# 0411tony/Yue

Measured on AMD Instinct MI355X. Metric: BPR triplet-updates/sec at k=128 (S-round semantics, user rows sequential; the reference's exact sequential semantics: secondary.exact), higher is better.
Workload: dtype f32

## Files before the change

yue_amd/csrc/bpr_device.hpp:

```cpp
#pragma once
#include <hip/hip_runtime.h>
#include <stdint.h>

namespace yue {

constexpr int kNllSlots = 1024;
constexpr int kMaxAttempts = 64;

struct TrainArgs {
    float *P, *Q, *dP, *dQ;
    float *stage;
#ifdef YUE_STAMPS
    unsigned long long *stamps;
#endif
    const int32_t *ev_u, *ev_i;
    int32_t *ev_j;
    const int64_t *indptr;
    const int32_t *indices;
    double *nll_slots;
    int64_t m, n;
    int k;
    float ru, ri;
    double lr;
    uint64_t seed;
// ... 76 lines not shown
    const double r8 = r4 * r4;
    const double c0 = __builtin_fma(b1, r4, b0), c1 = __builtin_fma(a6, r4, b2);
    return __builtin_ldexp(__builtin_fma(c1, r8, c0), (int)n);
}
__device__ __forceinline__ double chain_rcp(double d) {
    double y = __builtin_amdgcn_rcp(d);
    double e = __builtin_fma(-d, y, 1.0);
    y = __builtin_fma(e, y, y);
    e = __builtin_fma(-d, y, 1.0);
    y = __builtin_fma(e, y, y);
    e = __builtin_fma(-d, y, 1.0);
    return __builtin_fma(e, y, y);
}

__device__ __forceinline__ double chain_sigmoid(float x) {
    const double xd = (double)x;
    if (__builtin_fabs(xd) <= 700.0) return chain_rcp(1.0 + chain_exp(-xd));
    return 1.0 / (1.0 + exp(-xd));
}
__device__ __forceinline__ float chain_coef_fast(float x, float lr) {
    return lr * __builtin_amdgcn_rcpf(1.0f + __builtin_amdgcn_exp2f(x * 1.44269502162933349609375f));
}

__device__ __forceinline__ float wave_sum_any(float v) {
    v = v + dpp_mov<0xB1>(v);
    v = v + dpp_mov<0x4E>(v);
    v = v + dpp_mov<0x141>(v);
    v = v + dpp_mov<0x140>(v);
    v = v + __builtin_bit_cast(float, __builtin_amdgcn_update_dpp(0, __builtin_bit_cast(int, v), 0x142, 0xA, 0xF, false));
    v = v + __builtin_bit_cast(float, __builtin_amdgcn_update_dpp(0, __builtin_bit_cast(int, v), 0x143, 0xC, 0xF, false));
    return rdlane(v, 63);
}

struct Elem { float p2, qi2, qj2; };
__device__ __forceinline__ Elem bpr_elem(float p, float qi, float qj, float c, float ru, float ri) {
    const float d = qi - qj;
    const float td = c * d;
    const float p1 = p + td;
    const float tq = c * p1;
    const float qi1 = qi + tq;
    const float qj1 = qj - tq;
    const float rp = ru * p1;
    const float ra = ri * qi1;
    const float rb = ri * qj1;
    Elem o;
    o.p2 = p1 - rp;
    o.qi2 = qi1 - ra;
    o.qj2 = qj1 - rb;
    return o;
}

#define YUE_BLOAD(rs, vo, so) __builtin_bit_cast(float, __builtin_amdgcn_raw_buffer_load_b32((rs), (vo), (so), 0))
#define YUE_BSTORE(val, rs, vo, so) __builtin_amdgcn_raw_buffer_store_b32(__builtin_bit_cast(unsigned, (val)), (rs), (vo), (so), 0)
#define YUE_BLOAD_SC1(rs, vo, so) __builtin_bit_cast(float, __builtin_amdgcn_raw_buffer_load_b32((rs), (vo), (so), 16))
#define YUE_BSTORE_SC1(val, rs, vo, so) __builtin_amdgcn_raw_buffer_store_b32(__builtin_bit_cast(unsigned, (val)), (rs), (vo), (so), 16)
#define YUE_BATOMIC(val, rs, vo, so) __builtin_amdgcn_raw_ptr_buffer_atomic_fadd_f32((val), (rs), (vo), (so), 0)
#ifdef YUE_STAMPS
#define YUE_STAMP(ix, waits) do { asm volatile(waits ::: "memory"); if (a.stamps && lane == 0) a.stamps[(size_t)wave * 8 + (ix)] = wall_clock64(); } while (0)
#else
#define YUE_STAMP(ix, waits) do {} while (0)
#endif
constexpr unsigned kOobOffset = 0x80000000u;
constexpr unsigned long long kTouch = 0x100000001ull;
constexpr int kRsrcFlags = 0x00020000;
constexpr unsigned kStageMax = 4;

constexpr int kHeaderSlack = 16;
template <int TPW>
struct __attribute__((aligned(4))) HeaderBlock { int32_t w[TPW]; };

}
```

yue_amd/csrc/bpr_host.hip:

```cpp
#include "host_common.hpp"

#include "train_kernels.hpp"
#include "round_kernels.hpp"

using yue_host::fail;
using yue_host::kr_of;
static_assert(yue::kNllSlots == yue_host::kNllSlotsHost && yue::kHeaderSlack == yue_host::kHeaderSlackHost, "host_common.hpp mirrors these");

namespace {

yue::TrainArgs make_args(yue_ctx *c, double lr, double regU, double regI) {
    yue::TrainArgs a{};
    a.P = c->P.p; a.Q = c->Q.p; a.dP = c->dP.p; a.dQ = c->dQ.p;
    a.stage = c->Q.p ? c->Q.p + (size_t)c->n * c->k : nullptr;
    a.ev_u = c->ev_u.p; a.ev_i = c->ev_i.p; a.ev_j = c->ev_j.p;
    a.indptr = c->indptr.p; a.indices = c->indices.p;
    a.nll_slots = c->scal.p;
    a.m = c->m; a.n = c->n; a.k = c->k;
    a.lr = lr;
    a.ru = (float)(lr * regU);
    a.ri = (float)(lr * regI);
    a.neg_lo = 0; a.neg_range = (int32_t)c->n;
    return a;
}
// ... 110 lines not shown
    if (c->h_bounds != bounds) {
        HIPCHK(hipStreamSynchronize(c->stream));
        c->h_bounds = bounds;
        HIPCHK(hipMemcpyAsync(c->d_bounds.p, c->h_bounds.data(), (size_t)(R + 1) * sizeof(int64_t), hipMemcpyHostToDevice, c->stream));
    }
    HIPCHK(hipMemsetAsync(c->round_rows.p, 0, (size_t)R * sizeof(unsigned long long), c->stream));
    HIPCHK(c->fold.resize((size_t)(E + 4 * R + 8)));
    yue::MetaArgs ma{};
    ma.ev_i = a.ev_i; ma.ev_j = a.ev_j; ma.bounds = c->d_bounds.p; ma.R = R; ma.n = (int32_t)c->n;
    const bool bucketed = meta_bucketed(c);
    if (bucketed) {
        ma.range = 1 << yue::kBucketShift;
        ma.G = (int32_t)((c->n + ma.range - 1) >> yue::kBucketShift);
        HIPCHK(c->bk_touch.resize((size_t)(2 * E + 2))); HIPCHK(c->bk_ptr.resize((size_t)R * (ma.G + 1)));
        yue::BucketArgs ba{};
        ba.ev_i = a.ev_i; ba.ev_j = a.ev_j; ba.bounds = c->d_bounds.p; ba.R = R; ba.G = ma.G;
        ba.bk_touch = c->bk_touch.p; ba.bk_ptr = c->bk_ptr.p; ba.meta_i = c->meta_i.p; ba.meta_j = c->meta_j.p;
        int cus0 = 0;
        HIPCHK(hipDeviceGetAttribute(&cus0, hipDeviceAttributeMultiprocessorCount, c->device));
        hipLaunchKernelGGL(yue::k_round_bucket, dim3((unsigned)std::min<int64_t>(R, 2 * cus0)), dim3(1024), 0, c->stream, ba);
        ma.bk_touch = c->bk_touch.p; ma.bk_ptr = c->bk_ptr.p;
    } else {
        ma.G = (int32_t)((c->n + kMetaRangeMax - 1) / kMetaRangeMax);
        ma.range = (int32_t)((c->n + ma.G - 1) / ma.G);
    }
    ma.chunk = (ma.range + 1023) / 1024; ma.chunk |= 1;
    int64_t widest = 0;
    for (int64_t r = 0; r < R; ++r) widest = std::max(widest, bounds[(size_t)r + 1] - bounds[(size_t)r]);
    const double mean_touches = 2.0 * (double)widest / (double)std::max<int64_t>(1, c->n);
    const uint32_t stage_auto = (uint32_t)std::min<double>((double)yue::kMetaStageMax, std::max<double>((double)yue::kMetaStageDefault,
                                                         std::ceil(mean_touches * (kr_of(c->k) == 1 ? 4.0 : 2.0))));
    ma.stage_max = !c->staged ? 1u : c->opt_round_stage >= 2 ? (uint32_t)c->opt_round_stage : stage_auto;
    c->last_stage_max = (int)ma.stage_max;
    ma.meta_i = c->meta_i.p; ma.meta_j = c->meta_j.p; ma.round_rows = c->round_rows.p; ma.fold = c->fold.p;
    const size_t lds = (size_t)ma.range * sizeof(uint32_t);
    const void *kfn = bucketed ? (const void *)yue::k_round_meta<true> : (const void *)yue::k_round_meta<false>;
    HIPCHK(hipFuncSetAttribute(kfn, hipFuncAttributeMaxDynamicSharedMemorySize, (int)lds));
    int per_cu = 0, cus = 0;
    if (bucketed) { HIPCHK(hipOccupancyMaxActiveBlocksPerMultiprocessor(&per_cu, yue::k_round_meta<true>, 1024, lds)); }
    else { HIPCHK(hipOccupancyMaxActiveBlocksPerMultiprocessor(&per_cu, yue::k_round_meta<false>, 1024, lds)); }
    HIPCHK(hipDeviceGetAttribute(&cus, hipDeviceAttributeMultiprocessorCount, c->device));
    const int64_t grid = std::max<int64_t>(8, std::min<int64_t>((R * ma.G + 7) / 8 * 8, (int64_t)std::max(per_cu, 1) * cus / 8 * 8));
    if (bucketed) hipLaunchKernelGGL(yue::k_round_meta<true>, dim3((unsigned)grid), dim3(1024), lds, c->stream, ma);
    else
        hipLaunchKernelGGL(yue::k_round_meta<false>, dim3((unsigned)grid), dim3(1024), lds, c->stream, ma);
    HIPCHK(hipGetLastError());
    return YUE_OK;
}

void launch_round_fold(yue_ctx *c, const yue::TrainArgs &a, int64_t e0, int64_t e1, int64_t round_index) {
    yue::FoldArgs f{};
    f.fold = c->fold.p + yue::fold_base(e0, round_index); f.round_rows = c->round_rows.p + round_index; f.Q = a.Q; f.dQ = a.dQ; f.stage = a.stage; f.k = c->k; f.capacity = (uint32_t)((e1 - e0) & ~(int64_t)3);
    const dim3 fgrid((unsigned)std::min<int64_t>(c->opt_fold_blocks, std::max<int64_t>(1, (e1 - e0 + 15) / 16))), block(256);
    switch (kr_of(c->k)) {
        case 1: hipLaunchKernelGGL(yue::k_round_fold<1>, fgrid, block, 0, c->stream, f); break;
        case 2: hipLaunchKernelGGL(yue::k_round_fold<2>, fgrid, block, 0, c->stream, f); break;
        default: hipLaunchKernelGGL(yue::k_round_fold<4>, fgrid, block, 0, c->stream, f); break;
    }
}

int launch_round_m(yue_ctx *c, const yue::TrainArgs &a_in, int64_t e0, int64_t e1, int64_t round_index) {
    yue::RoundMArgs ra{};
    ra.e_begin = e0; ra.e_end = e1; ra.staged = c->staged ? 1 : 0;
    const int tpw = tpw_of(c, true);
    const int64_t waves = (e1 - e0 + tpw - 1) / tpw;
    const int64_t blocks = (waves + 3) / 4;
    if (blocks == 0) return YUE_OK;
    const dim3 grid((unsigned)blocks), block(256);
#ifdef YUE_STAMPS
    yue::TrainArgs a = a_in;
    a.stamps = nullptr;
    if (c->update_launches++ == c->stamp_launch) {
        HIPCHK(c->stamps.resize((size_t)waves * 8));
        HIPCHK(hipMemsetAsync(c->stamps.p, 0, (size_t)waves * 64, c->stream));
        a.stamps = c->stamps.p;
        c->stamp_waves = waves;
    }
#else
    const yue::TrainArgs &a = a_in;
#endif
    const uint32_t *mi = c->meta_i.p, *mj = c->meta_j.p;
    if (c->bigq) {
        switch (kr_of(c->k) * 16 + tpw) {
            case 1 * 16 + 8: hipLaunchKernelGGL((yue::k_round_m<1, 8, true>), grid, block, 0, c->stream, a, ra, a.ev_u, a.ev_i, a.ev_j, mi, mj); break;
            case 2 * 16 + 8: hipLaunchKernelGGL((yue::k_round_m<2, 8, true>), grid, block, 0, c->stream, a, ra, a.ev_u, a.ev_i, a.ev_j, mi, mj); break;
// ... 619 lines not shown
```

yue_amd/csrc/core_host.hip:

```cpp
#include "host_common.hpp"

namespace yue_host {
thread_local std::string g_err;
int fail(int code, const std::string &msg) { g_err = msg; return code; }
}
using yue_host::fail;
void yue_comm_release(yue_ctx *c);

extern "C" {

const char *yue_last_error(void) { return yue_host::g_err.c_str(); }
int yue_version(void) { return 1; }

int yue_ctx_create(int device, yue_ctx **out) {
    if (!out) return fail(YUE_ERR_ARG, "yue_ctx_create: out is NULL");
    int ndev = 0;
    HIPCHK(hipGetDeviceCount(&ndev));
    if (ndev <= 0) return fail(YUE_ERR_HIP, "no HIP device visible: libyue_hip needs an MI355X (no CPU fallback exists)");
    if (device < 0 || device >= ndev) return fail(YUE_ERR_ARG, "device ordinal out of range");
    HIPCHK(hipSetDevice(device));
    yue_ctx *c = new yue_ctx();
    c->device = device;
    const auto init = [c]() -> int {
        HIPCHK(hipStreamCreateWithFlags(&c->stream, hipStreamNonBlocking));
// ... 2 lines not shown
        HIPCHK(hipEventCreateWithFlags(&c->ev_comm, hipEventDisableTiming));
        HIPCHK(hipEventCreate(&c->ev_t_rounds));
        HIPCHK(hipEventCreate(&c->ev_t_comm));
        HIPCHK(hipEventCreate(&c->ev_scan0));
        HIPCHK(hipEventCreate(&c->ev_scan1));
        HIPCHK(c->scal.resize(yue_host::kNllSlotsHost + 8));
        return YUE_OK;
    };
    const int rc = init();
    if (rc) { const std::string msg = yue_host::g_err; (void)yue_ctx_destroy(c); yue_host::g_err = msg; return rc; }
    *out = c;
    return YUE_OK;
}

int yue_ctx_destroy(yue_ctx *c) {
    if (!c) return YUE_OK;
    (void)hipSetDevice(c->device);
    if (c->stream) (void)hipStreamSynchronize(c->stream);
    if (c->comm_stream) (void)hipStreamSynchronize(c->comm_stream);
    yue_comm_release(c);
    if (c->comm_stream) (void)hipStreamDestroy(c->comm_stream);
    if (c->ev_rounds) (void)hipEventDestroy(c->ev_rounds);
    if (c->ev_comm) (void)hipEventDestroy(c->ev_comm);
    if (c->ev_t_rounds) (void)hipEventDestroy(c->ev_t_rounds);
    if (c->ev_t_comm) (void)hipEventDestroy(c->ev_t_comm);
    if (c->ev_scan0) (void)hipEventDestroy(c->ev_scan0);
    if (c->ev_chain0) (void)hipEventDestroy(c->ev_chain0);
    if (c->ev_chain1) (void)hipEventDestroy(c->ev_chain1);
    if (c->ev_scan1) (void)hipEventDestroy(c->ev_scan1);
    for (auto &pr : c->ev_pool) { (void)hipEventDestroy(pr.first); (void)hipEventDestroy(pr.second); }
    c->P.release(); c->Q.release(); c->dP.release(); c->dQ.release(); c->margins.release();
    c->cnt0.release(); c->cnt1.release(); c->cntp0.release(); c->cntp1.release();
    c->tab0.release(); c->tab1.release();
    c->meta_i.release(); c->meta_j.release(); c->round_rows.release(); c->d_bounds.release(); c->fold.release(); c->bk_touch.release(); c->bk_ptr.release();
    c->ev_u.release(); c->ev_i.release(); c->ev_j.release(); c->indices.release(); c->indptr.release();
    c->xu.release(); c->xi.release(); c->xj.release(); c->xk.release(); c->x_loss.release(); c->scal.release();
    c->aU_m.release(); c->aU_v.release(); c->aV_m.release(); c->aV_v.release();
    c->s_users.release(); c->s_ids.release(); c->s_mask_idx.release(); c->s_flags.release();
    c->s_mask_ptr.release(); c->s_scores.release(); c->s_row.release(); c->s_norms.release(); c->s_work.release(); c->s_qb.release(); c->s_masks.release(); c->s_few.release(); c->s_few_ids.release(); c->s_few_scores.release();
    c->fP.release(); c->fBi.release(); c->f_coef.release(); c->f_x.release(); c->f_hist.release(); c->f_scores.release();
    c->f_out_sc.release(); c->fQ.release(); c->f_ptr.release(); c->f_items.release(); c->f_negs.release(); c->f_ids.release(); c->f_flags.release();
    c->f_uq_ptr.release(); c->f_neg_ptr.release(); c->f_uq_items.release(); c->f_loc_i.release(); c->f_loc_j.release();
    c->f_wq.release(); c->f_dQ.release(); c->f_wp.release(); c->f_wb.release(); c->f_dP.release(); c->f_dB.release();
    c->ch_key.release(); c->ch_val.release(); c->ch_key2.release(); c->ch_val2.release(); c->ch_seg.release(); c->ch_ord_i.release(); c->ch_ord_j.release();
    c->ch_head.release(); c->ch_incl.release(); c->ch_ord_u.release(); c->ch_rkey.release(); c->ch_rval.release(); c->ch_run_ptr.release(); c->d_ev_ptr.release();
    c->ch_run_u.release(); c->ch_tmp.release(); c->ch_Qv.release(); c->ch_Pv.release(); c->ch_ctl.release(); c->ch_stats.release();
    yue_host::wrmf_release(c);
    yue_host::knn_release(c);
    if (c->stream) (void)hipStreamDestroy(c->stream);
    delete c;
    return YUE_OK;
}

int yue_sync(yue_ctx *c) {
    if (!c) return fail(YUE_ERR_ARG, "null context");
    HIPCHK(hipSetDevice(c->device));
    HIPCHK(hipStreamSynchronize(c->stream));
    return YUE_OK;
}

int yue_set_factors(yue_ctx *c, const float *P, int64_t m, const float *Q, int64_t n, int k) {
    if (!c || !P || !Q) return fail(YUE_ERR_ARG, "yue_set_factors: null argument");
    if (m <= 0 || n <= 0 || k <= 0 || k > 256) return fail(YUE_ERR_ARG, "yue_set_factors: need m,n > 0 and 1 <= k <= 256");
    if (n >= (1ll << 31) || m >= (1ll << 31)) return fail(YUE_ERR_ARG, "yue_set_factors: ids must fit int32");
    HIPCHK(hipSetDevice(c->device));
    if (c->have_inter && (m != c->m || n != c->n || k != c->k)) c->have_inter = false;
    if (k != c->k) c->opt_round_tpw = 0;
// ... 69 lines not shown
```

yue_amd/csrc/host_common.hpp:

```cpp
#pragma once
#include "../../include/yue_hip.h"

#include <hip/hip_runtime.h>

#include <algorithm>
#include <cmath>
#include <cstdio>
#include <cstdlib>
#include <cstring>
#include <string>
#include <vector>

struct ncclComm;
struct yue_wrmf;
struct yue_knn;

namespace yue_host {

int fail(int code, const std::string &msg);

#define HIPCHK(expr)                                                                              \
    do {                                                                                          \
        hipError_t e_ = (expr);                                                                   \
        if (e_ != hipSuccess)                                                                     \
// ... 8 lines not shown
        if (count <= n && p) return hipSuccess;
        if (p) { hipError_t e = hipFree(p); p = nullptr; n = 0; if (e != hipSuccess) return e; }
        if (count == 0) return hipSuccess;
        hipError_t e = hipMalloc((void **)&p, count * sizeof(T));
        if (e == hipSuccess) n = count;
        return e;
    }
    void release() { if (p) (void)hipFree(p); p = nullptr; n = 0; }
};

constexpr int kNllSlotsHost = 1024;
constexpr int kHeaderSlackHost = 16;

inline int kr_of(int k) { return k <= 64 ? 1 : k <= 128 ? 2 : 4; }

}

using yue_host::DevBuf;

struct yue_ctx {
    int device = 0;
    hipStream_t stream = nullptr;
    int64_t m = 0, n = 0, E = 0, nnz = 0;
    int k = 0;
    bool have_factors = false, have_inter = false;
    DevBuf<float> P, Q, dP, dQ;
    DevBuf<float> margins;
    DevBuf<unsigned long long> cnt0, cnt1;
    DevBuf<uint32_t> cntp0, cntp1;
    DevBuf<uint32_t> tab0, tab1;
    bool staged = false;
    bool bigq = false;
    DevBuf<uint32_t> meta_i, meta_j;
    DevBuf<unsigned long long> round_rows;
    DevBuf<uint2> fold, bk_touch;
    DevBuf<uint32_t> bk_ptr;
    DevBuf<int64_t> d_bounds;
    std::vector<int64_t> h_bounds;
#ifdef YUE_STAMPS
    DevBuf<unsigned long long> stamps;
    int64_t stamp_launch = -1, update_launches = 0, stamp_waves = 0;
#endif
    DevBuf<int32_t> ev_u, ev_i, ev_j, indices;
    DevBuf<int64_t> indptr;
    DevBuf<int32_t> xu, xi, xj, xk;
    DevBuf<double> x_loss;
    DevBuf<float> aU_m, aU_v, aV_m, aV_v;
    int64_t adam_m = 0, adam_n = 0; int adam_k = 0;
    DevBuf<double> scal;
    std::vector<int64_t> h_ev_ptr;
    DevBuf<int32_t> s_users, s_ids, s_mask_idx, s_flags;
    DevBuf<int32_t> s_few, s_few_ids;
    DevBuf<float> s_few_scores;
    int64_t scan_few_users = 0;
    DevBuf<int64_t> s_mask_ptr;
    DevBuf<float> s_scores, s_row, s_norms;
    double scan_ms = 0.0;
    int64_t scan_events = 0, scan_rescored = 0, scan_tiles_done = 0, scan_tiles_total = 0;
    DevBuf<unsigned long long> s_work;
    DevBuf<unsigned short> s_qb;
    DevBuf<uint32_t> s_masks;
    int opt_scan_two_phase = 1;
    int64_t opt_scan_streams_min_users = 262144;
    int opt_scan_slabs = 4;
    int opt_scan_streams = 2;
    int opt_scan_filter_ub = 3;
// ... 87 lines not shown
```

yue_amd/csrc/round_kernels.hpp:

```cpp
#pragma once
#include "train_kernels.hpp"

#ifdef YUE_ABL_NO_HOT
#define YUE_M_HOT(val, rs, vo, so) asm volatile("" :: "v"(val))
#else
#define YUE_M_HOT(val, rs, vo, so) YUE_BATOMIC(val, rs, vo, so)
#endif
#ifdef YUE_ABL_NO_DP
#define YUE_M_DP(val, rs, vo, so) asm volatile("" :: "v"(val))
#else
#define YUE_M_DP(val, rs, vo, so) YUE_BATOMIC(val, rs, vo, so)
#endif

#define YUE_BLOAD_NT(rs, vo, so) __builtin_bit_cast(float, __builtin_amdgcn_raw_buffer_load_b32((rs), (vo), (so), 2))
#if defined(YUE_EXP_LOAD_CACHED)
#define YUE_M_LOAD_J(rs, vo, so) YUE_BLOAD(rs, vo, so)
#define YUE_M_LOAD_I(rs, vo, so) YUE_BLOAD(rs, vo, so)
#elif defined(YUE_EXP_LOAD_NT)
#define YUE_M_LOAD_J(rs, vo, so) YUE_BLOAD_NT(rs, vo, so)
#define YUE_M_LOAD_I(rs, vo, so) YUE_BLOAD_NT(rs, vo, so)
#else
#define YUE_M_LOAD_J(rs, vo, so) YUE_BLOAD_NT(rs, vo, so)
#define YUE_M_LOAD_I(rs, vo, so) YUE_BLOAD(rs, vo, so)
#endif

#define YUE_FOLD_LD(p) __builtin_nontemporal_load(p)
#define YUE_FOLD_LDROW(p) (*(p))

namespace yue {

constexpr uint32_t kMetaStageMax = 64u;
constexpr uint32_t kMetaStageDefault = 4u;
constexpr uint32_t kMetaUnique = 1u, kMetaStaged = 2u, kMetaHot = 3u;
constexpr int kMetaUnroll = 8;
__host__ __device__ inline uint32_t meta_kind(uint32_t w) { return w & 3u; }
__host__ __device__ inline uint32_t meta_slot(uint32_t w) { return w >> 2; }
__host__ __device__ inline uint32_t fold_count(uint32_t w) { return w >> 25; }
__host__ __device__ inline uint32_t fold_block(uint32_t w) { return w & 0x1ffffffu; }

struct MetaArgs {
    const int32_t *ev_i, *ev_j;
    const int64_t *bounds;
    int64_t R;
    int32_t n;
    int32_t range;
    int32_t G;
    int32_t chunk;
    uint32_t stage_max;
    uint32_t *meta_i, *meta_j;
    unsigned long long *round_rows;
    uint2 *fold;
    const uint2 *bk_touch;
    const uint32_t *bk_ptr;
};

__host__ __device__ inline int64_t fold_base(int64_t e0, int64_t r) { return (e0 + 4 * r + 3) & ~(int64_t)3; }

template <bool BUCKETED>
__global__ void __launch_bounds__(1024) k_round_meta(MetaArgs a) {
    extern __shared__ uint32_t slots[];
    __shared__ unsigned long long wsum[16];
    __shared__ unsigned long long range_base;
    const int tid = threadIdx.x, lane = tid & 63, wv = tid >> 6;
    const int64_t xcd = blockIdx.x & 7, local = blockIdx.x >> 3, per_xcd = gridDim.x >> 3;
    const int64_t rounds_here = (a.R - xcd + 7) >> 3;
    for (int64_t sq = local; sq < rounds_here * a.G; sq += per_xcd) {
        const int64_t r = (sq / a.G) * 8 + xcd;
        const int32_t g = (int32_t)(sq % a.G);
        const int32_t lo = g * a.range;
        const int32_t width = min(a.range, a.n - lo);
        const int64_t e0 = a.bounds[r], e1 = a.bounds[r + 1];
        for (int s = tid; s < a.range; s += 1024) slots[s] = 0u;
        __syncthreads();
        const uint2 *mine_t = nullptr;
        uint32_t mine_n = 0u;
        if (BUCKETED) {
            const uint32_t *bp = a.bk_ptr + r * (a.G + 1) + g;
            mine_t = a.bk_touch + 2 * e0 + bp[0];
            mine_n = bp[1] - bp[0];
        }
        if (BUCKETED) {
            for (uint32_t t = tid; t < mine_n; t += 1024) atomicAdd(&slots[mine_t[t].x - (uint32_t)lo], 1u);
// ... 18 lines not shown
        const int s0 = tid * a.chunk;
        unsigned long long mine = 0ull;
        for (int q = 0; q < a.chunk; ++q) {
            const int s = s0 + q;
            if (s < width) { const uint32_t c = slots[s]; if (c >= 2u) mine += (1ull << 32) + (c <= a.stage_max ? c : 0u); }
        }
        unsigned long long incl = mine;
#pragma unroll
        for (int off = 1; off < 64; off <<= 1) { const unsigned long long up = __shfl_up(incl, off); if (lane >= off) incl += up; }
        if (lane == 63) wsum[wv] = incl;
        __syncthreads();
        if (tid == 0) {
            unsigned long long total = 0ull;
            for (int q = 0; q < 16; ++q) total += wsum[q];
            range_base = total ? atomicAdd(a.round_rows + r, total) : 0ull;
        }
        __syncthreads();
        unsigned long long run = range_base + incl - mine;
        for (int q = 0; q < wv; ++q) run += wsum[q];
        uint2 *fold = a.fold + fold_base(e0, r);
        for (int q = 0; q < a.chunk; ++q) {
            const int s = s0 + q;
            if (s < width) {
                const uint32_t c = slots[s];
                if (c >= 2u) {
                    const bool st = c <= a.stage_max;
                    slots[s] = st ? (kMetaStaged | ((uint32_t)run << 2)) : kMetaHot;
                    fold[run >> 32] = make_uint2((uint32_t)(lo + s), st ? ((c << 25) | ((uint32_t)run & 0x1ffffffu)) : 0u);
                    run += (1ull << 32) + (st ? c : 0u);
                }
            }
        }
        __syncthreads();
        if (BUCKETED) {
            for (uint32_t t = tid; t < mine_n; t += 1024) {
                const uint2 tc = mine_t[t];
                const uint32_t sl = tc.x - (uint32_t)lo;
                const uint32_t wd = slots[sl];
                const uint32_t mw = meta_kind(wd) == kMetaStaged ? atomicAdd(&slots[sl], 4u) : wd;
                ((tc.y & 1u) ? a.meta_j : a.meta_i)[e0 + (tc.y >> 1)] = mw;
            }
        } else
        for (int64_t eb = e0 + tid; eb < e1; eb += 1024 * kMetaUnroll) {
            int32_t vi[kMetaUnroll], vj[kMetaUnroll];
#pragma unroll
            for (int q = 0; q < kMetaUnroll; ++q) {
                const int64_t e = eb + 1024 * q;
                vj[q] = e < e1 ? a.ev_j[e] : -1; vi[q] = e < e1 ? a.ev_i[e] : 0;
            }
#pragma unroll
            for (int q = 0; q < kMetaUnroll; ++q) {
                const int64_t e = eb + 1024 * q;
                if (vj[q] >= 0) {
                    const uint32_t si = (uint32_t)(vi[q] - lo), sj = (uint32_t)(vj[q] - lo);
                    if (si < (uint32_t)width) {
                        const uint32_t wd = slots[si];
                        a.meta_i[e] = meta_kind(wd) == kMetaStaged ? atomicAdd(&slots[si], 4u) : wd;
                    }
                    if (sj < (uint32_t)width) {
                        const uint32_t wd = slots[sj];
                        a.meta_j[e] = meta_kind(wd) == kMetaStaged ? atomicAdd(&slots[sj], 4u) : wd;
                    }
                } else if (g == 0 && e < e1) {
                    a.meta_i[e] = 0u; a.meta_j[e] = 0u;
                }
            }
        }
        __syncthreads();
    }
}

constexpr int kBucketShift = 15;
constexpr int kBucketRangesMax = 256;
struct BucketArgs {
    const int32_t *ev_i, *ev_j;
    const int64_t *bounds;
    int64_t R;
    int32_t G;
    uint2 *bk_touch;
    uint32_t *bk_ptr;
    uint32_t *meta_i, *meta_j;
};

__global__ void __launch_bounds__(1024) k_round_bucket(BucketArgs a) {
    __shared__ uint32_t cnt[kBucketRangesMax], off[kBucketRangesMax + 1];
    const int tid = threadIdx.x;
    for (int64_t r = blockIdx.x; r < a.R; r += gridDim.x) {
        const int64_t e0 = a.bounds[r], e1 = a.bounds[r + 1];
        for (int g = tid; g < a.G; g += 1024) cnt[g] = 0u;
        __syncthreads();
        for (int64_t eb = e0 + tid; eb < e1; eb += 1024 * kMetaUnroll) {
            int32_t vi[kMetaUnroll], vj[kMetaUnroll];
#pragma unroll
            for (int q = 0; q < kMetaUnroll; ++q) {
                const int64_t e = eb + 1024 * q;
// ... 118 lines not shown
#pragma unroll
        for (int r = 0; r < KR; ++r) p[t][r] = YUE_BLOAD(rsP, vo[r], ou[t]);

    YUE_STAMP(2, "s_waitcnt vmcnt(0)");
    float xs = 0.0f;
#pragma unroll
    for (int t = 0; t < TPW; ++t) {
        float ai = 0.0f, aj = 0.0f;
#pragma unroll
        for (int r = 0; r < KR; ++r) {
            const float a1 = p[t][r] * qi[t][r]; ai = ai + a1;
            const float a2 = p[t][r] * qj[t][r]; aj = aj + a2;
        }
        const float x = wave_sum(ai) - wave_sum(aj);
        xs = lane == t ? x : xs;
    }
    __builtin_amdgcn_sched_barrier(0);
    const double s = 1.0 / (1.0 + exp(-(double)xs));
    const float cs = (float)(a.lr * (1.0 - s));
    double nll = (lane < TPW && j >= 0) ? -log(s) : 0.0;
    __builtin_amdgcn_sched_barrier(0);

    YUE_STAMP(3, "");
    float dp[KR];
#pragma unroll
    for (int r = 0; r < KR; ++r) dp[r] = 0.0f;
    bool run_ok = false;
#pragma unroll
    for (int t = 0; t < TPW; ++t) {
        const float c = rdlane(cs, t);
        const unsigned cli = meta_kind(hmi[t]), clj = meta_kind(hmj[t]);
        const bool uniq_i = cli == kMetaUnique, uniq_j = clj == kMetaUnique;
        const bool hot_i = cli == kMetaHot, hot_j = clj == kMetaHot;
        const unsigned wi = uniq_i ? oi[t] : stage0 + meta_slot(hmi[t]) * row_bytes;
        const unsigned wj = uniq_j ? oj[t] : stage0 + meta_slot(hmj[t]) * row_bytes;
        if (ok[t]) {
            run_ok = true;
            Elem o[KR];
#pragma unroll
            for (int r = 0; r < KR; ++r) { o[r] = bpr_elem(p[t][r], qi[t][r], qj[t][r], c, a.ru, a.ri); dp[r] += o[r].p2 - p[t][r]; }
            if (BIGQ) {
                const uint64_t ri_ = (uint64_t)(unsigned)hi_[t] * k, rj_ = (uint64_t)(unsigned)hj[t] * k;
                float *di = hot_i ? a.dQ + ri_ : uniq_i ? a.Q + ri_ : a.stage + (uint64_t)meta_slot(hmi[t]) * k;
                float *dj = hot_j ? a.dQ + rj_ : uniq_j ? a.Q + rj_ : a.stage + (uint64_t)meta_slot(hmj[t]) * k;
#pragma unroll
                for (int r = 0; r < KR; ++r) {
                    if (ev[r]) {
                        if (hot_i) unsafeAtomicAdd(di + el[r], o[r].qi2 - qi[t][r]); else di[el[r]] = uniq_i ? o[r].qi2 : o[r].qi2 - qi[t][r];
                        if (hot_j) unsafeAtomicAdd(dj + el[r], o[r].qj2 - qj[t][r]); else dj[el[r]] = uniq_j ? o[r].qj2 : o[r].qj2 - qj[t][r];
                    }
                }
            } else {
            if (!hot_i) {
#pragma unroll
                for (int r = 0; r < KR; ++r) YUE_BSTORE(uniq_i ? o[r].qi2 : o[r].qi2 - qi[t][r], rsQ, vo[r], wi);
            } else {
#pragma unroll
                for (int r = 0; r < KR; ++r) YUE_M_HOT(o[r].qi2 - qi[t][r], rsdQ, vo[r], oi[t]);
            }
            if (!hot_j) {
#pragma unroll
                for (int r = 0; r < KR; ++r) YUE_BSTORE(uniq_j ? o[r].qj2 : o[r].qj2 - qj[t][r], rsQ, vo[r], wj);
            } else {
#pragma unroll
                for (int r = 0; r < KR; ++r) YUE_M_HOT(o[r].qj2 - qj[t][r], rsdQ, vo[r], oj[t]);
            }
            }
        }
        const bool exists = base + t < ra.e_end;
        const bool last = exists && ((t == TPW - 1) || base + t + 1 >= ra.e_end || ru_[t + 1 < TPW ? t + 1 : t] != ru_[t]);
        if (last) {
            if (run_ok) {
#pragma unroll
                for (int r = 0; r < KR; ++r) YUE_M_DP(dp[r], rsdP, vo[r], ou[t]);
            }
#pragma unroll
            for (int r = 0; r < KR; ++r) dp[r] = 0.0f;
            run_ok = false;
        }
        __builtin_amdgcn_sched_barrier(0);
    }
    YUE_STAMP(4, ""); YUE_STAMP(5, ""); YUE_STAMP(6, "");
#pragma unroll
    for (int off = 1; off < TPW; off <<= 1) nll += __shfl_xor(nll, off);
    if (lane == 0 && nll != 0.0) atomicAdd(a.nll_slots + (wave & (kNllSlots - 1)), nll);
    YUE_STAMP(7, "s_waitcnt vmcnt(0)");
}

struct RoundUArgs {
    int64_t u_begin, u_end;
    const int64_t *ev_ptr;
    int64_t e_begin, e_end;
    int staged;
    float *margins;
};

template <int KR, bool FAST>
__global__ void __launch_bounds__(256) k_round_u(TrainArgs a, RoundUArgs ra, const int32_t *__restrict__ evi, const int32_t *__restrict__ evj,
// ... 2 lines not shown
    const int64_t wave = (int64_t)blockIdx.x * 4 + __builtin_amdgcn_readfirstlane((int)(threadIdx.x >> 6));
    const int64_t u = ra.u_begin + wave;
    if (u >= ra.u_end) return;
    const int64_t e0 = ra.ev_ptr[u], e1 = ra.ev_ptr[u + 1];
    if (e1 <= e0) return;
    const unsigned k = (unsigned)a.k;
    const unsigned row_bytes = k * 4u;
    unsigned vo[KR];
#pragma unroll
    for (int r = 0; r < KR; ++r) { const unsigned e = 64u * r + lane; vo[r] = e < k ? e * 4u : kOobOffset; }
    const uint64_t qbytes = (uint64_t)a.n * row_bytes;
    const int qrec = (int)(qbytes < 0x7fffffffull ? qbytes : 0x7fffffffull);
    const unsigned stage0 = (unsigned)a.n * row_bytes;
    const uint64_t qsbytes = qbytes + (ra.staged ? 2ull * (uint64_t)(ra.e_end - ra.e_begin) * row_bytes : 0ull);
    const int qsrec = (int)(qsbytes < 0x7fffffffull ? qsbytes : 0x7fffffffull);
    const auto rsQ = __builtin_amdgcn_make_buffer_rsrc(a.Q, 0, qsrec, kRsrcFlags);
    const auto rsdQ = __builtin_amdgcn_make_buffer_rsrc(a.dQ, 0, qrec, kRsrcFlags);
    float *prow = a.P + (uint64_t)u * k;
    float p[KR];
#pragma unroll
    for (int r = 0; r < KR; ++r) { const unsigned e = 64u * r + lane; p[r] = e < k ? prow[e] : 0.0f; }
    const float lrf = (float)a.lr;
    const unsigned len = (unsigned)(e1 - e0 < 0x7fffffff ? e1 - e0 : 0x7fffffff);
    for (unsigned seg = 0; seg < len; seg += 64u) {
        int hI, hJ;
        uint32_t hMI, hMJ;
        {
            const bool ex = seg + (unsigned)lane < len;
            const int64_t e = e0 + seg + (ex ? lane : 0);
            hI = evi[e]; hJ = evj[e]; hMI = mti[e]; hMJ = mtj[e];
            if (!ex) { hI = 0; hJ = -1; hMI = 0u; hMJ = 0u; }
        }
        const unsigned seg_len = len - seg < 64u ? len - seg : 64u;
        float xs = 0.0f;
        auto gather = [&](float (&qi)[KR], float (&qj)[KR], unsigned t) {
            const int ti = __builtin_amdgcn_readlane(hI, t), tj = __builtin_amdgcn_readlane(hJ, t);
            const unsigned oi = (unsigned)ti * row_bytes, oj = (unsigned)(tj < 0 ? 0 : tj) * row_bytes;
#pragma unroll
            for (int r = 0; r < KR; ++r) { qi[r] = YUE_M_LOAD_I(rsQ, vo[r], oi); qj[r] = YUE_M_LOAD_J(rsQ, vo[r], oj); }
        };
        auto step = [&](const float (&qi)[KR], const float (&qj)[KR], unsigned t) {
            const int tj = __builtin_amdgcn_readlane(hJ, t);
            if (tj < 0) return;
            const int ti = __builtin_amdgcn_readlane(hI, t);
            const uint32_t mi = (uint32_t)__builtin_amdgcn_readlane((int)hMI, t), mj = (uint32_t)__builtin_amdgcn_readlane((int)hMJ, t);
            float ai = 0.0f, aj = 0.0f;
#pragma unroll
            for (int r = 0; r < KR; ++r) { const float a1 = p[r] * qi[r]; ai = ai + a1; const float a2 = p[r] * qj[r]; aj = aj + a2; }
            const float x = wave_sum(ai) - wave_sum(aj);
            const float c = FAST ? chain_coef_fast(x, lrf) : (float)(a.lr * (1.0 - chain_sigmoid(x)));
            xs = (unsigned)lane == t ? x : xs;
            const unsigned cli = meta_kind(mi), clj = meta_kind(mj);
            const bool uniq_i = cli == kMetaUnique, uniq_j = clj == kMetaUnique;
            const unsigned oi = (unsigned)ti * row_bytes, oj = (unsigned)tj * row_bytes;
            const unsigned wi = uniq_i ? oi : stage0 + meta_slot(mi) * row_bytes;
            const unsigned wj = uniq_j ? oj : stage0 + meta_slot(mj) * row_bytes;
            Elem o[KR];
#pragma unroll
            for (int r = 0; r < KR; ++r) { o[r] = bpr_elem(p[r], qi[r], qj[r], c, a.ru, a.ri); p[r] = o[r].p2; }
            if (cli != kMetaHot) {
#pragma unroll
                for (int r = 0; r < KR; ++r) YUE_BSTORE(uniq_i ? o[r].qi2 : o[r].qi2 - qi[r], rsQ, vo[r], wi);
            } else {
#pragma unroll
                for (int r = 0; r < KR; ++r) YUE_M_HOT(o[r].qi2 - qi[r], rsdQ, vo[r], oi);
            }
            if (clj != kMetaHot) {
#pragma unroll
                for (int r = 0; r < KR; ++r) YUE_BSTORE(uniq_j ? o[r].qj2 : o[r].qj2 - qj[r], rsQ, vo[r], wj);
            } else {
#pragma unroll
                for (int r = 0; r < KR; ++r) YUE_M_HOT(o[r].qj2 - qj[r], rsdQ, vo[r], oj);
            }
        };
        constexpr int D = KR == 1 ? 8 : 4;
        float qi[D][KR], qj[D][KR];
#pragma unroll
        for (int s_ = 0; s_ < D; ++s_) gather(qi[s_], qj[s_], (unsigned)s_);
        for (unsigned t = 0; t < seg_len; t += D) {
#pragma unroll
            for (int s_ = 0; s_ < D; ++s_) {
                step(qi[s_], qj[s_], t + s_);
                gather(qi[s_], qj[s_], (t + s_ + D) & 63u);
            }
        }
        if ((unsigned)lane < seg_len) ra.margins[e0 + seg + lane] = xs;
    }
#pragma unroll
    for (int r = 0; r < KR; ++r) { const unsigned e = 64u * r + lane; if (e < k) prow[e] = p[r]; }
}

__global__ void __launch_bounds__(256) k_loss_margins(const float *__restrict__ x, const int32_t *__restrict__ evj, int64_t E, double *nll_slots) {
    double nl = 0.0;
    const int64_t stride = (int64_t)gridDim.x * blockDim.x;
    for (int64_t e = (int64_t)blockIdx.x * blockDim.x + threadIdx.x; e < E; e += stride)
        if (evj[e] >= 0) nl += -log(chain_sigmoid(x[e]));
#pragma unroll
    for (int off = 1; off < 64; off <<= 1) nl += __shfl_xor(nl, off);
    if ((threadIdx.x & 63) == 0 && nl != 0.0) atomicAdd(nll_slots + ((blockIdx.x * 4 + (threadIdx.x >> 6)) & (kNllSlots - 1)), nl);
}

struct FoldArgs {
    const uint2 *fold;
    const unsigned long long *round_rows;
    float *Q, *dQ;
    const float *stage;
    int k;
    uint32_t capacity;
};

template <int KR, int EPG>
__device__ __forceinline__ void fold_group(const FoldArgs &f, int lane, unsigned k, uint32_t nact, const uint2 (&ent)[4]) {
    float x[EPG][KR], st[EPG][4][KR];
    unsigned el[KR];
    bool big = false;
#pragma unroll
    for (int r = 0; r < KR; ++r) el[r] = min(64u * r + lane, k - 1u);
#pragma unroll
    for (int sl = 0; sl < EPG; ++sl) {
        if ((uint32_t)sl >= nact) continue;
        const uint32_t c = fold_count(ent[sl].y);
        const bool hot = c == 0u;
        const float *row = f.Q + (uint64_t)ent[sl].x * k;
        const float *src = hot ? f.dQ + (uint64_t)ent[sl].x * k : f.stage + (uint64_t)fold_block(ent[sl].y) * k;
#pragma unroll
        for (int r = 0; r < KR; ++r) { st[sl][0][r] = YUE_FOLD_LD(src + el[r]); if (!hot) st[sl][1][r] = YUE_FOLD_LD(src + (uint64_t)k + el[r]); }
        if (c > 2u) {
#pragma unroll
            for (unsigned q = 2; q < 4; ++q)
#pragma unroll
                for (int r = 0; r < KR; ++r) st[sl][q][r] = YUE_FOLD_LD(src + (uint64_t)(q < c ? q : 0u) * k + el[r]);
        }
        big = big || c > 4u;
#pragma unroll
        for (int r = 0; r < KR; ++r) x[sl][r] = YUE_FOLD_LDROW(row + el[r]);
    }
#pragma unroll
    for (int sl = 0; sl < EPG; ++sl) {
        if ((uint32_t)sl >= nact) continue;
        const uint32_t c = fold_count(ent[sl].y);
        const bool hot = c == 0u;
        float *row = f.Q + (uint64_t)ent[sl].x * k;
        float *dr = f.dQ + (uint64_t)ent[sl].x * k;
#pragma unroll
        for (int r = 0; r < KR; ++r) {
            const unsigned e = 64u * r + lane;
            float acc = st[sl][0][r];
#pragma unroll
            for (unsigned q = 1; q < 4; ++q) { const float v = q < c ? st[sl][q][r] : 0.0f; acc = acc + v; }
            st[sl][0][r] = acc;
            if (c <= 4u && e < k) { row[e] = x[sl][r] + acc; if (hot) dr[e] = 0.0f; }
        }
    }
    if (big) {
#pragma unroll
        for (int sl = 0; sl < EPG; ++sl) {
            if ((uint32_t)sl >= nact) continue;
            const uint32_t c = fold_count(ent[sl].y);
            if (c <= 4u) continue;
            const float *src = f.stage + (uint64_t)fold_block(ent[sl].y) * k;
            float *row = f.Q + (uint64_t)ent[sl].x * k;
            float acc[KR];
#pragma unroll
            for (int r = 0; r < KR; ++r) acc[r] = st[sl][0][r];
            constexpr unsigned STEP = KR == 1 ? 8u : 4u;
            for (uint32_t q0 = 4u; q0 < c; q0 += STEP) {
                float v[STEP][KR];
#pragma unroll
                for (unsigned q = 0; q < STEP; ++q)
#pragma unroll
                    for (int r = 0; r < KR; ++r) v[q][r] = YUE_FOLD_LD(src + (uint64_t)(q0 + q < c ? q0 + q : q0) * k + el[r]);
#pragma unroll
                for (unsigned q = 0; q < STEP; ++q)
#pragma unroll
                    for (int r = 0; r < KR; ++r) acc[r] = acc[r] + (q0 + q < c ? v[q][r] : 0.0f);
            }
#pragma unroll
            for (int r = 0; r < KR; ++r) { const unsigned e = 64u * r + lane; if (e < k) row[e] = x[sl][r] + acc[r]; }
        }
    }
}

template <int KR>
__global__ void __launch_bounds__(256) k_round_fold(FoldArgs f) {
    constexpr int EPG = KR == 4 ? 2 : 4;
    const int lane = threadIdx.x & 63;
    const uint32_t wave = blockIdx.x * 4u + (uint32_t)__builtin_amdgcn_readfirstlane((int)(threadIdx.x >> 6));
    const uint32_t nwaves = gridDim.x * 4u;
    const unsigned k = (unsigned)f.k;
    const uint32_t b0 = wave * EPG;
    uint2 ent[4];
    typedef uint32_t u32x8 __attribute__((ext_vector_type(8)));
    u32x8 ev;
    unsigned long long cntw;
    const bool spec = b0 + 4u <= f.capacity;
    const uint2 *first = f.fold + (spec ? b0 : 0u);
    asm volatile("s_load_dwordx8 %0, %2, 0x0\n\ts_load_dwordx2 %1, %3, 0x0\n\ts_waitcnt lgkmcnt(0)"
                 : "=&s"(ev), "=&s"(cntw) : "s"(first), "s"(f.round_rows) : "memory");
    const uint32_t cnt = (uint32_t)(cntw >> 32);
    ent[0] = make_uint2(ev[0], ev[1]); ent[1] = make_uint2(ev[2], ev[3]); ent[2] = make_uint2(ev[4], ev[5]); ent[3] = make_uint2(ev[6], ev[7]);
    if (b0 < cnt) {
        if (!spec) {
#pragma unroll
            for (int sl = 0; sl < EPG; ++sl) ent[sl] = f.fold[b0 + sl < cnt ? b0 + sl : b0];
        }
        fold_group<KR, EPG>(f, lane, k, min((uint32_t)EPG, cnt - b0), ent);
    }
    for (uint32_t b = b0 + nwaves * EPG; b < cnt; b += nwaves * EPG) {
// ... 8 lines not shown
```

Measured before the change: 1.749 billion.

## Stage one shared tq row per triplet and recompute item deltas during fold

Each triplet whose positive or negative item is staged now writes a single shared tq row to a step-indexed stage slot, instead of a separate delta row per touched item. A new stage_idx buffer is filled in the meta kernel and records which step, and which side (i or j), produced each touch. The fold kernel reads those refs, gathers the tq rows, and rebuilds each item delta from the start-of-round Q row and ri. The aim is to cut stage write traffic and slot bookkeeping, in exchange for index writes, indirect gathers and extra arithmetic in the fold.

```diff
diff --git a/yue_amd/csrc/bpr_device.hpp b/yue_amd/csrc/bpr_device.hpp
--- a/yue_amd/csrc/bpr_device.hpp
+++ b/yue_amd/csrc/bpr_device.hpp
@@ -132,21 +132,24 @@
     return rdlane(v, 63);
 }
 
-struct Elem { float p2, qi2, qj2; };
+__device__ __forceinline__ float item_step(float q, float tq, bool neg, float ri) {
+    const float q1 = neg ? q - tq : q + tq;
+    const float rq = ri * q1;
+    return q1 - rq;
+}
+
+struct Elem { float p2, qi2, qj2, tq; };
 __device__ __forceinline__ Elem bpr_elem(float p, float qi, float qj, float c, float ru, float ri) {
     const float d = qi - qj;
     const float td = c * d;
     const float p1 = p + td;
     const float tq = c * p1;
-    const float qi1 = qi + tq;
-    const float qj1 = qj - tq;
     const float rp = ru * p1;
-    const float ra = ri * qi1;
-    const float rb = ri * qj1;
     Elem o;
     o.p2 = p1 - rp;
-    o.qi2 = qi1 - ra;
-    o.qj2 = qj1 - rb;
+    o.qi2 = item_step(qi, tq, false, ri);
+    o.qj2 = item_step(qj, tq, true, ri);
+    o.tq = tq;
     return o;
 }
 
diff --git a/yue_amd/csrc/bpr_host.hip b/yue_amd/csrc/bpr_host.hip
--- a/yue_amd/csrc/bpr_host.hip
+++ b/yue_amd/csrc/bpr_host.hip
@@ -166,7 +166,8 @@
                                                          std::ceil(mean_touches * (kr_of(c->k) == 1 ? 4.0 : 2.0))));
     ma.stage_max = !c->staged ? 1u : c->opt_round_stage >= 2 ? (uint32_t)c->opt_round_stage : stage_auto;
     c->last_stage_max = (int)ma.stage_max;
-    ma.meta_i = c->meta_i.p; ma.meta_j = c->meta_j.p; ma.round_rows = c->round_rows.p; ma.fold = c->fold.p;
+    if (ma.stage_max > 1u) HIPCHK(c->stage_idx.resize((size_t)(2 * E)));
+    ma.meta_i = c->meta_i.p; ma.meta_j = c->meta_j.p; ma.round_rows = c->round_rows.p; ma.fold = c->fold.p; ma.stage_idx = c->stage_idx.p;
     const size_t lds = (size_t)ma.range * sizeof(uint32_t);
     const void *kfn = bucketed ? (const void *)yue::k_round_meta<true> : (const void *)yue::k_round_meta<false>;
     HIPCHK(hipFuncSetAttribute(kfn, hipFuncAttributeMaxDynamicSharedMemorySize, (int)lds));
@@ -185,6 +186,7 @@
 void launch_round_fold(yue_ctx *c, const yue::TrainArgs &a, int64_t e0, int64_t e1, int64_t round_index) {
     yue::FoldArgs f{};
     f.fold = c->fold.p + yue::fold_base(e0, round_index); f.round_rows = c->round_rows.p + round_index; f.Q = a.Q; f.dQ = a.dQ; f.stage = a.stage; f.k = c->k; f.capacity = (uint32_t)((e1 - e0) & ~(int64_t)3);
+    f.idx = c->stage_idx.p ? c->stage_idx.p + 2 * e0 : nullptr; f.idx_bytes = c->stage_idx.p ? (uint32_t)(8 * (e1 - e0)) : 0u; f.ri = a.ri;
     const dim3 fgrid((unsigned)std::min<int64_t>(c->opt_fold_blocks, std::max<int64_t>(1, (e1 - e0 + 15) / 16))), block(256);
     switch (kr_of(c->k)) {
         case 1: hipLaunchKernelGGL(yue::k_round_fold<1>, fgrid, block, 0, c->stream, f); break;
diff --git a/yue_amd/csrc/core_host.hip b/yue_amd/csrc/core_host.hip
--- a/yue_amd/csrc/core_host.hip
+++ b/yue_amd/csrc/core_host.hip
@@ -58,7 +58,7 @@
     c->P.release(); c->Q.release(); c->dP.release(); c->dQ.release(); c->margins.release();
     c->cnt0.release(); c->cnt1.release(); c->cntp0.release(); c->cntp1.release();
     c->tab0.release(); c->tab1.release();
-    c->meta_i.release(); c->meta_j.release(); c->round_rows.release(); c->d_bounds.release(); c->fold.release(); c->bk_touch.release(); c->bk_ptr.release();
+    c->meta_i.release(); c->meta_j.release(); c->stage_idx.release(); c->round_rows.release(); c->d_bounds.release(); c->fold.release(); c->bk_touch.release(); c->bk_ptr.release();
     c->ev_u.release(); c->ev_i.release(); c->ev_j.release(); c->indices.release(); c->indptr.release();
     c->xu.release(); c->xi.release(); c->xj.release(); c->xk.release(); c->x_loss.release(); c->scal.release();
     c->aU_m.release(); c->aU_v.release(); c->aV_m.release(); c->aV_v.release();
diff --git a/yue_amd/csrc/host_common.hpp b/yue_amd/csrc/host_common.hpp
--- a/yue_amd/csrc/host_common.hpp
+++ b/yue_amd/csrc/host_common.hpp
@@ -64,6 +64,7 @@
     bool staged = false;
     bool bigq = false;
     DevBuf<uint32_t> meta_i, meta_j;
+    DevBuf<uint32_t> stage_idx;
     DevBuf<unsigned long long> round_rows;
     DevBuf<uint2> fold, bk_touch;
     DevBuf<uint32_t> bk_ptr;
diff --git a/yue_amd/csrc/round_kernels.hpp b/yue_amd/csrc/round_kernels.hpp
--- a/yue_amd/csrc/round_kernels.hpp
+++ b/yue_amd/csrc/round_kernels.hpp
@@ -48,6 +48,7 @@
     int32_t chunk;
     uint32_t stage_max;
     uint32_t *meta_i, *meta_j;
+    uint32_t *stage_idx;
     unsigned long long *round_rows;
     uint2 *fold;
     const uint2 *bk_touch;
@@ -132,13 +133,17 @@
             }
         }
         __syncthreads();
+        uint32_t *idx = a.stage_idx + 2 * e0;
+        auto touch_word = [&](uint32_t sl, uint32_t ref) -> uint32_t {
+            const uint32_t wd = slots[sl];
+            if (meta_kind(wd) != kMetaStaged) return wd;
+            idx[meta_slot(atomicAdd(&slots[sl], 4u))] = ref;
+            return kMetaStaged | (ref << 2);
+        };
         if (BUCKETED) {
             for (uint32_t t = tid; t < mine_n; t += 1024) {
                 const uint2 tc = mine_t[t];
-                const uint32_t sl = tc.x - (uint32_t)lo;
-                const uint32_t wd = slots[sl];
-                const uint32_t mw = meta_kind(wd) == kMetaStaged ? atomicAdd(&slots[sl], 4u) : wd;
-                ((tc.y & 1u) ? a.meta_j : a.meta_i)[e0 + (tc.y >> 1)] = mw;
+                ((tc.y & 1u) ? a.meta_j : a.meta_i)[e0 + (tc.y >> 1)] = touch_word(tc.x - (uint32_t)lo, tc.y);
             }
         } else
         for (int64_t eb = e0 + tid; eb < e1; eb += 1024 * kMetaUnroll) {
@@ -153,14 +158,9 @@
                 const int64_t e = eb + 1024 * q;
                 if (vj[q] >= 0) {
                     const uint32_t si = (uint32_t)(vi[q] - lo), sj = (uint32_t)(vj[q] - lo);
-                    if (si < (uint32_t)width) {
-                        const uint32_t wd = slots[si];
-                        a.meta_i[e] = meta_kind(wd) == kMetaStaged ? atomicAdd(&slots[si], 4u) : wd;
-                    }
-                    if (sj < (uint32_t)width) {
-                        const uint32_t wd = slots[sj];
-                        a.meta_j[e] = meta_kind(wd) == kMetaStaged ? atomicAdd(&slots[sj], 4u) : wd;
-                    }
+                    const uint32_t ref = (uint32_t)(e - e0) << 1;
+                    if (si < (uint32_t)width) a.meta_i[e] = touch_word(si, ref);
+                    if (sj < (uint32_t)width) a.meta_j[e] = touch_word(sj, ref | 1u);
                 } else if (g == 0 && e < e1) {
                     a.meta_i[e] = 0u; a.meta_j[e] = 0u;
                 }
@@ -345,8 +345,8 @@
         const unsigned cli = meta_kind(hmi[t]), clj = meta_kind(hmj[t]);
         const bool uniq_i = cli == kMetaUnique, uniq_j = clj == kMetaUnique;
         const bool hot_i = cli == kMetaHot, hot_j = clj == kMetaHot;
-        const unsigned wi = uniq_i ? oi[t] : stage0 + meta_slot(hmi[t]) * row_bytes;
-        const unsigned wj = uniq_j ? oj[t] : stage0 + meta_slot(hmj[t]) * row_bytes;
+        const bool step_row = cli == kMetaStaged || clj == kMetaStaged;
+        const unsigned ws = stage0 + (unsigned)(base + t - ra.e_begin) * row_bytes;
         if (ok[t]) {
             run_ok = true;
             Elem o[KR];
@@ -354,29 +354,33 @@
             for (int r = 0; r < KR; ++r) { o[r] = bpr_elem(p[t][r], qi[t][r], qj[t][r], c, a.ru, a.ri); dp[r] += o[r].p2 - p[t][r]; }
             if (BIGQ) {
                 const uint64_t ri_ = (uint64_t)(unsigned)hi_[t] * k, rj_ = (uint64_t)(unsigned)hj[t] * k;
-                float *di = hot_i ? a.dQ + ri_ : uniq_i ? a.Q + ri_ : a.stage + (uint64_t)meta_slot(hmi[t]) * k;
-                float *dj = hot_j ? a.dQ + rj_ : uniq_j ? a.Q + rj_ : a.stage + (uint64_t)meta_slot(hmj[t]) * k;
+                float *ds = a.stage + (uint64_t)(base + t - ra.e_begin) * k;
 #pragma unroll
                 for (int r = 0; r < KR; ++r) {
                     if (ev[r]) {
-                        if (hot_i) unsafeAtomicAdd(di + el[r], o[r].qi2 - qi[t][r]); else di[el[r]] = uniq_i ? o[r].qi2 : o[r].qi2 - qi[t][r];
-                        if (hot_j) unsafeAtomicAdd(dj + el[r], o[r].qj2 - qj[t][r]); else dj[el[r]] = uniq_j ? o[r].qj2 : o[r].qj2 - qj[t][r];
+                        if (hot_i) unsafeAtomicAdd(a.dQ + ri_ + el[r], o[r].qi2 - qi[t][r]); else if (uniq_i) a.Q[ri_ + el[r]] = o[r].qi2;
+                        if (hot_j) unsafeAtomicAdd(a.dQ + rj_ + el[r], o[r].qj2 - qj[t][r]); else if (uniq_j) a.Q[rj_ + el[r]] = o[r].qj2;
+                        if (step_row) ds[el[r]] = o[r].tq;
                     }
                 }
             } else {
-            if (!hot_i) {
-#pragma unroll
-                for (int r = 0; r < KR; ++r) YUE_BSTORE(uniq_i ? o[r].qi2 : o[r].qi2 - qi[t][r], rsQ, vo[r], wi);
-            } else {
+            if (uniq_i) {
+#pragma unroll
+                for (int r = 0; r < KR; ++r) YUE_BSTORE(o[r].qi2, rsQ, vo[r], oi[t]);
+            } else if (hot_i) {
 #pragma unroll
                 for (int r = 0; r < KR; ++r) YUE_M_HOT(o[r].qi2 - qi[t][r], rsdQ, vo[r], oi[t]);
             }
-            if (!hot_j) {
-#pragma unroll
-                for (int r = 0; r < KR; ++r) YUE_BSTORE(uniq_j ? o[r].qj2 : o[r].qj2 - qj[t][r], rsQ, vo[r], wj);
-            } else {
+            if (uniq_j) {
+#pragma unroll
+                for (int r = 0; r < KR; ++r) YUE_BSTORE(o[r].qj2, rsQ, vo[r], oj[t]);
+            } else if (hot_j) {
 #pragma unroll
                 for (int r = 0; r < KR; ++r) YUE_M_HOT(o[r].qj2 - qj[t][r], rsdQ, vo[r], oj[t]);
+            }
+            if (step_row) {
+#pragma unroll
+                for (int r = 0; r < KR; ++r) YUE_BSTORE(o[r].tq, rsQ, vo[r], ws);
             }
             }
         }
@@ -445,6 +449,7 @@
             if (!ex) { hI = 0; hJ = -1; hMI = 0u; hMJ = 0u; }
         }
         const unsigned seg_len = len - seg < 64u ? len - seg : 64u;
+        const unsigned step0 = (unsigned)(e0 - ra.e_begin) + seg;
         float xs = 0.0f;
         auto gather = [&](float (&qi)[KR], float (&qj)[KR], unsigned t) {
             const int ti = __builtin_amdgcn_readlane(hI, t), tj = __builtin_amdgcn_readlane(hJ, t);
@@ -464,26 +469,28 @@
             const float c = FAST ? chain_coef_fast(x, lrf) : (float)(a.lr * (1.0 - chain_sigmoid(x)));
             xs = (unsigned)lane == t ? x : xs;
             const unsigned cli = meta_kind(mi), clj = meta_kind(mj);
-            const bool uniq_i = cli == kMetaUnique, uniq_j = clj == kMetaUnique;
             const unsigned oi = (unsigned)ti * row_bytes, oj = (unsigned)tj * row_bytes;
-            const unsigned wi = uniq_i ? oi : stage0 + meta_slot(mi) * row_bytes;
-            const unsigned wj = uniq_j ? oj : stage0 + meta_slot(mj) * row_bytes;
             Elem o[KR];
 #pragma unroll
             for (int r = 0; r < KR; ++r) { o[r] = bpr_elem(p[r], qi[r], qj[r], c, a.ru, a.ri); p[r] = o[r].p2; }
-            if (cli != kMetaHot) {
-#pragma unroll
-                for (int r = 0; r < KR; ++r) YUE_BSTORE(uniq_i ? o[r].qi2 : o[r].qi2 - qi[r], rsQ, vo[r], wi);
-            } else {
+            if (cli == kMetaUnique) {
+#pragma unroll
+                for (int r = 0; r < KR; ++r) YUE_BSTORE(o[r].qi2, rsQ, vo[r], oi);
+            } else if (cli == kMetaHot) {
 #pragma unroll
                 for (int r = 0; r < KR; ++r) YUE_M_HOT(o[r].qi2 - qi[r], rsdQ, vo[r], oi);
             }
-            if (clj != kMetaHot) {
-#pragma unroll
-                for (int r = 0; r < KR; ++r) YUE_BSTORE(uniq_j ? o[r].qj2 : o[r].qj2 - qj[r], rsQ, vo[r], wj);
-            } else {
+            if (clj == kMetaUnique) {
+#pragma unroll
+                for (int r = 0; r < KR; ++r) YUE_BSTORE(o[r].qj2, rsQ, vo[r], oj);
+            } else if (clj == kMetaHot) {
 #pragma unroll
                 for (int r = 0; r < KR; ++r) YUE_M_HOT(o[r].qj2 - qj[r], rsdQ, vo[r], oj);
+            }
+            if (cli == kMetaStaged || clj == kMetaStaged) {
+                const unsigned ws = stage0 + (step0 + t) * row_bytes;
+#pragma unroll
+                for (int r = 0; r < KR; ++r) YUE_BSTORE(o[r].tq, rsQ, vo[r], ws);
             }
         };
         constexpr int D = KR == 1 ? 8 : 4;
@@ -516,37 +523,58 @@
 struct FoldArgs {
     const uint2 *fold;
     const unsigned long long *round_rows;
+    const uint32_t *idx;
+    uint32_t idx_bytes;
     float *Q, *dQ;
     const float *stage;
     int k;
+    float ri;
     uint32_t capacity;
 };
+
+__device__ __forceinline__ float fold_delta(float x, float tq, uint32_t w, float ri) { return item_step(x, tq, (w & 1u) != 0u, ri) - x; }
 
 template <int KR, int EPG>
 __device__ __forceinline__ void fold_group(const FoldArgs &f, int lane, unsigned k, uint32_t nact, const uint2 (&ent)[4]) {
     float x[EPG][KR], st[EPG][4][KR];
+    uint32_t iw[EPG], w[EPG][4];
     unsigned el[KR];
     bool big = false;
 #pragma unroll
     for (int r = 0; r < KR; ++r) el[r] = min(64u * r + lane, k - 1u);
+    const auto rsI = __builtin_amdgcn_make_buffer_rsrc(const_cast<uint32_t *>(f.idx), 0, (int)f.idx_bytes, kRsrcFlags);
+#pragma unroll
+    for (int sl = 0; sl < EPG; ++sl) {
+        const bool act = (uint32_t)sl < nact;
+        const uint32_t c = act ? fold_count(ent[sl].y) : 0u;
+        const unsigned vi = c != 0u ? (fold_block(ent[sl].y) + min((uint32_t)lane, c - 1u)) * 4u : kOobOffset;
+        iw[sl] = (uint32_t)__builtin_amdgcn_raw_buffer_load_b32(rsI, vi, 0, 0);
+        const float *row = f.Q + (uint64_t)(act ? ent[sl].x : ent[0].x) * k;
+#pragma unroll
+        for (int r = 0; r < KR; ++r) x[sl][r] = YUE_FOLD_LDROW(row + el[r]);
+    }
+#pragma unroll
+    for (int sl = 0; sl < EPG; ++sl)
+#pragma unroll
+        for (int q = 0; q < 4; ++q) w[sl][q] = (uint32_t)__builtin_amdgcn_readlane((int)iw[sl], q);
 #pragma unroll
     for (int sl = 0; sl < EPG; ++sl) {
         if ((uint32_t)sl >= nact) continue;
         const uint32_t c = fold_count(ent[sl].y);
         const bool hot = c == 0u;
-        const float *row = f.Q + (uint64_t)ent[sl].x * k;
-        const float *src = hot ? f.dQ + (uint64_t)ent[sl].x * k : f.stage + (uint64_t)fold_block(ent[sl].y) * k;
-#pragma unroll
-        for (int r = 0; r < KR; ++r) { st[sl][0][r] = YUE_FOLD_LD(src + el[r]); if (!hot) st[sl][1][r] = YUE_FOLD_LD(src + (uint64_t)k + el[r]); }
+        const float *s0 = hot ? f.dQ + (uint64_t)ent[sl].x * k : f.stage + (uint64_t)(w[sl][0] >> 1) * k;
+        const float *s1 = f.stage + (uint64_t)(w[sl][1] >> 1) * k;
+#pragma unroll
+        for (int r = 0; r < KR; ++r) { st[sl][0][r] = YUE_FOLD_LD(s0 + el[r]); if (!hot) st[sl][1][r] = YUE_FOLD_LD(s1 + el[r]); }
         if (c > 2u) {
 #pragma unroll
-            for (unsigned q = 2; q < 4; ++q)
-#pragma unroll
-                for (int r = 0; r < KR; ++r) st[sl][q][r] = YUE_FOLD_LD(src + (uint64_t)(q < c ? q : 0u) * k + el[r]);
+            for (unsigned q = 2; q < 4; ++q) {
+                const float *sq = f.stage + (uint64_t)(w[sl][q < c ? q : 0u] >> 1) * k;
+#pragma unroll
+                for (int r = 0; r < KR; ++r) st[sl][q][r] = YUE_FOLD_LD(sq + el[r]);
+            }
         }
         big = big || c > 4u;
-#pragma unroll
-        for (int r = 0; r < KR; ++r) x[sl][r] = YUE_FOLD_LDROW(row + el[r]);
     }
 #pragma unroll
     for (int sl = 0; sl < EPG; ++sl) {
@@ -558,9 +586,9 @@
 #pragma unroll
         for (int r = 0; r < KR; ++r) {
             const unsigned e = 64u * r + lane;
-            float acc = st[sl][0][r];
-#pragma unroll
-            for (unsigned q = 1; q < 4; ++q) { const float v = q < c ? st[sl][q][r] : 0.0f; acc = acc + v; }
+            float acc = hot ? st[sl][0][r] : fold_delta(x[sl][r], st[sl][0][r], w[sl][0], f.ri);
+#pragma unroll
+            for (unsigned q = 1; q < 4; ++q) { const float v = q < c ? fold_delta(x[sl][r], st[sl][q][r], w[sl][q], f.ri) : 0.0f; acc = acc + v; }
             st[sl][0][r] = acc;
             if (c <= 4u && e < k) { row[e] = x[sl][r] + acc; if (hot) dr[e] = 0.0f; }
         }
@@ -571,7 +599,6 @@
             if ((uint32_t)sl >= nact) continue;
             const uint32_t c = fold_count(ent[sl].y);
             if (c <= 4u) continue;
-            const float *src = f.stage + (uint64_t)fold_block(ent[sl].y) * k;
             float *row = f.Q + (uint64_t)ent[sl].x * k;
             float acc[KR];
 #pragma unroll
@@ -579,14 +606,18 @@
             constexpr unsigned STEP = KR == 1 ? 8u : 4u;
             for (uint32_t q0 = 4u; q0 < c; q0 += STEP) {
                 float v[STEP][KR];
+                uint32_t w[STEP];
+#pragma unroll
+                for (unsigned q = 0; q < STEP; ++q) {
+                    w[q] = (uint32_t)__builtin_amdgcn_readlane((int)iw[sl], (int)(q0 + q < c ? q0 + q : q0));
+                    const float *sq = f.stage + (uint64_t)(w[q] >> 1) * k;
+#pragma unroll
+                    for (int r = 0; r < KR; ++r) v[q][r] = YUE_FOLD_LD(sq + el[r]);
+                }
 #pragma unroll
                 for (unsigned q = 0; q < STEP; ++q)
 #pragma unroll
-                    for (int r = 0; r < KR; ++r) v[q][r] = YUE_FOLD_LD(src + (uint64_t)(q0 + q < c ? q0 + q : q0) * k + el[r]);
-#pragma unroll
-                for (unsigned q = 0; q < STEP; ++q)
-#pragma unroll
-                    for (int r = 0; r < KR; ++r) acc[r] = acc[r] + (q0 + q < c ? v[q][r] : 0.0f);
+                    for (int r = 0; r < KR; ++r) acc[r] = acc[r] + (q0 + q < c ? fold_delta(x[sl][r], v[q][r], w[q], f.ri) : 0.0f);
             }
 #pragma unroll
             for (int r = 0; r < KR; ++r) { const unsigned e = 64u * r + lane; if (e < k) row[e] = x[sl][r] + acc[r]; }
```

New measurement: 1.762 billion, median of 6. No clear change (+0.7%).
